# NethermindEth/cairo_zstd

Hardware: NVIDIA B200
Metric: decompressed GB/s (device-timed, whole box) at 1/2/4/8 B200; % of HBM roofline (higher is better)
Workload: dtype u8

## Files before the change

cairo_zstd_b200/csrc/czb_internal.cuh:

```cuda
#pragma once
#include <cuda_runtime.h>
#include <stdint.h>

#include "../../include/cairo_zstd_b200.h"


namespace czb {

constexpr uint32_t NONE32 = 0xFFFFFFFFu;
constexpr uint32_t MAX_BLOCK_SIZE = 128u * 1024u;
constexpr uint64_t MAX_FRAME_OUT = 0x0FFFFFFEull;

enum : uint8_t { BT_RAW = 0, BT_RLE = 1, BT_COMPRESSED = 2, BT_ERROR = 3 };
enum : uint8_t { LT_RAW = 0, LT_RLE = 1, LT_COMPRESSED = 2, LT_TREELESS = 3 };
enum : uint8_t { MODE_PREDEFINED = 0, MODE_RLE = 1, MODE_FSE = 2, MODE_REPEAT = 3 };

struct FrameInfo {
    int32_t status;
    uint32_t hdr_len;
    uint64_t fcs;
    uint64_t window;
    uint8_t descriptor;
    uint8_t has_checksum;
    uint16_t pad0;
    uint32_t checksum;
    uint32_t n_blocks;
    uint32_t n_huf;
    uint32_t n_fse;
    uint32_t size_cls;
    uint64_t lit_bytes;
    uint64_t n_seq;
    uint64_t n_seq_true;
    uint64_t src_end;
    uint32_t block_base;
    uint32_t fse_cls;
};

struct __align__(16) BlockDesc {
    uint32_t frame;
    uint32_t src_off;
    uint32_t size;
    uint8_t type;
    uint8_t last;
    uint8_t lit_type;
    uint8_t n_streams;
    int32_t pre_status;
    int32_t seqhdr_status;
    uint32_t regen;
    uint32_t lit_src_off;
    uint32_t lit_comp;
    uint32_t huf_src_blk;
    uint64_t lit_off;
    uint32_t n_seq;
    uint32_t seq_src_off;
    uint32_t seq_src_len;
    uint8_t modes;
    uint8_t first_in_frame;
    uint16_t pad;
    uint64_t seq_off;
    uint32_t tbl_src_blk[3];
    int32_t huf_status;
    int32_t fse_status;
    uint32_t hist_out[3];
    uint32_t out_bytes;
    uint32_t ml_sum;
};
static_assert(sizeof(BlockDesc) == 112, "BlockDesc layout");
constexpr uint32_t SEQ_ALIGN = 4;
__host__ __device__ inline uint64_t seq_slots(uint64_t n_seq) { return (n_seq + SEQ_ALIGN - 1) & ~(uint64_t)(SEQ_ALIGN - 1); }

typedef unsigned long long Seq;
constexpr uint32_t OFF29_CLAMP = (1u << 28) - 1u;
__host__ __device__ inline uint32_t seq_ll(Seq r) { return (uint32_t)r & 0x1FFFFu; }
__host__ __device__ inline uint32_t seq_ml(Seq r) { return (uint32_t)(r >> 17) & 0x3FFFFu; }
__host__ __device__ inline uint32_t seq_off29(Seq r) { return (uint32_t)(r >> 35); }

constexpr uint32_t SYM_BASE = 0xF0000000u;
constexpr uint32_t SYM_MID = 0x00800000u;
constexpr uint32_t REAL_OFF_CLAMP = 0xEFFFFFFFu;
__host__ __device__ inline uint32_t sym_enc(uint32_t k) { return SYM_BASE + (k << 24) + SYM_MID; }
__host__ __device__ inline bool sym_is(uint32_t v) { return v >= SYM_BASE; }
__host__ __device__ inline uint32_t sym_resolve(uint32_t v, uint32_t h0, uint32_t h1, uint32_t h2) {
    uint32_t t = v - SYM_BASE;
    uint32_t k = t >> 24;
    uint32_t c = SYM_MID - (t & 0x00FFFFFFu);
    uint32_t base = k == 0 ? h0 : (k == 1 ? h1 : h2);
    return base - c;
}
__host__ __device__ inline uint32_t off29_pack(uint32_t v) {
    if (v >= SYM_BASE) { uint32_t t = v - SYM_BASE; return (1u << 28) | ((t >> 24) << 24) | (SYM_MID - (t & 0x00FFFFFFu)); }
    return v < OFF29_CLAMP ? v : OFF29_CLAMP;
}
__host__ __device__ inline uint32_t off29_resolve(uint32_t f, uint32_t h0, uint32_t h1, uint32_t h2) {
    if (f >> 28) { uint32_t k = (f >> 24) & 3u, c = f & 0x00FFFFFFu; return (k == 0 ? h0 : (k == 1 ? h1 : h2)) - c; }
    return f;
}

struct FrameResume {
    uint32_t start_block;
    uint32_t h0, h1, h2;
    uint64_t out0;
    uint64_t bytes_read0;
};

struct WaveCounters {
    unsigned long long n_blocks, lit_bytes, n_seq;
    unsigned int n_huf, n_fse;
    unsigned int n_huf_cls[2];
    unsigned int exec_next;
    unsigned int pad[3];
    unsigned int frame_fill[32];
    unsigned int fse_fill[32];
};

struct HufRec {
    uint8_t weights[256];
    uint16_t nw;
    uint8_t max_bits;
    uint8_t pad;
    uint32_t tree_bytes;
    int32_t status;
    uint32_t blk;
};

struct WaveTotals {
    unsigned long long n_blocks, lit_bytes, n_seq, n_huf, n_fse, src_bytes;
    unsigned int frame_cls[32], fse_cls[32];
};
__host__ __device__ inline uint32_t size_class(uint64_t v) {
    uint32_t c = 0;
    while (v > 1 && c < 31) { v >>= 1; c++; }
    return c;
}

struct RevBits {
    const uint32_t* w0;
    uint32_t lo_mask;
    int wi;
    int avail;
    int rem;
    uint32_t wnext;
    uint64_t buf;

    __device__ __forceinline__ uint32_t load_word(int i) const {
        uint32_t w = 0;
        if (i >= 0) { w = w0[i]; if (i == 0) w &= lo_mask; }
        return w;
    }
    __device__ __forceinline__ void topup() {
        const uint32_t w = wi == -1 ? (wnext & lo_mask) : wnext;
        buf |= (uint64_t)w << (32 - avail);
        avail += 32;
        wnext = 0;
        if (wi >= 0) {
            wnext = w0[wi];
            if (wi >= 32) asm volatile("prefetch.global.L1 [%0];" ::"l"(w0 + wi - 32));
        }
        wi--;
    }
    __device__ __forceinline__ void topup_if_low() { if (avail <= 32) topup(); }
    __device__ __forceinline__ bool init(const uint8_t* p, int n) {
        rem = n * 8; avail = 0; buf = 0; wnext = 0; wi = -3; w0 = nullptr; lo_mask = 0;
        if (n <= 0) return false;
        const uintptr_t a0 = reinterpret_cast<uintptr_t>(p), a_last = a0 + (uintptr_t)n - 1;
        w0 = reinterpret_cast<const uint32_t*>(a0 & ~uintptr_t(3));
        lo_mask = 0xFFFFFFFFu << ((uint32_t)(a0 & 3) * 8);
        const int wl = (int)((a_last - reinterpret_cast<uintptr_t>(w0)) >> 2);
        const uint32_t v = (uint32_t)(a_last & 3) + 1;
        uint32_t w = load_word(wl) << ((4 - v) * 8);
        buf = (uint64_t)w << 32;
        avail = (int)(8 * v);
        wnext = wl - 1 >= 0 ? w0[wl - 1] : 0u;
        wi = wl - 2;
        topup();
        const uint32_t top = (uint32_t)(buf >> 56);
        if (top == 0) return false;
        const int pad = __clz(top) - 24 + 1;
        buf <<= pad; avail -= pad; rem -= pad;
        return true;
    }
    __device__ __forceinline__ uint32_t peek(int n) const {
        return (uint32_t)((buf >> 1) >> (63 - n));
    }
    __device__ __forceinline__ void skip(int n) { buf <<= n; avail -= n; rem -= n; }
    __device__ __forceinline__ uint32_t get(int n) { uint32_t v = peek(n); skip(n); return v; }
    __device__ __forceinline__ uint32_t get_safe(int n) { if (avail < n) topup(); return get(n); }
};

__device__ __forceinline__ void cp_async16(uint32_t smem_addr, const void* g) {
    asm volatile("cp.async.cg.shared.global [%0], [%1], 16;" ::"r"(smem_addr), "l"(g) : "memory");
}
__device__ __forceinline__ void cp_async16_if(bool pred, uint32_t smem_addr, const void* g) {
    asm volatile("{\n\t.reg .pred p;\n\tsetp.ne.u32 p, %2, 0;\n\t@p cp.async.cg.shared.global [%0], [%1], 16;\n\t}" ::"r"(smem_addr), "l"(g), "r"((uint32_t)pred) : "memory");
}
__device__ __forceinline__ void cp_async16_sz(uint32_t smem_addr, const void* g, uint32_t src_bytes) {
    asm volatile("cp.async.cg.shared.global [%0], [%1], 16, %2;" ::"r"(smem_addr), "l"(g), "r"(src_bytes) : "memory");
}
__device__ __forceinline__ void cp_async_commit() { asm volatile("cp.async.commit_group;" ::: "memory"); }
template <int N>
__device__ __forceinline__ void cp_async_wait() { asm volatile("cp.async.wait_group %0;" ::"n"(N) : "memory"); }
__device__ __forceinline__ uint32_t lds32(uint32_t smem_addr) {
    uint32_t v;
    asm volatile("ld.shared.u32 %0, [%1];" : "=r"(v) : "r"(smem_addr) : "memory");
    return v;
}

__device__ __forceinline__ uint32_t shr_clamp(uint32_t x, uint32_t n) {
    uint32_t v;
    asm("shr.b32 %0, %1, %2;" : "=r"(v) : "r"(x), "r"(n));
    return v;
}
template <int RING_BYTES, int WAIT>
struct RevBitsWinT {
    static constexpr int RING = RING_BYTES;
    static constexpr int WAIT_GROUPS = WAIT;
    const uint8_t* c_lo;
    uint32_t ring;
    int P;
    int start;
    int chunk;

    __device__ __forceinline__ int rem() const { return P - start; }
    __device__ __forceinline__ uint32_t window() const {
        const uint32_t wo = ((uint32_t)P >> 5) << 2;
        const uint32_t hi = lds32(ring + (wo & (RING - 1))), lo = lds32(ring + ((wo - 4u) & (RING - 1)));
        return __funnelshift_r(lo, hi, (uint32_t)P & 31u);
    }
    struct Raw { uint32_t lo, hi, sh; };
    __device__ __forceinline__ Raw window_raw() const {
        const uint32_t wo = ((uint32_t)P >> 5) << 2;
        Raw r;
        r.hi = lds32(ring + (wo & (RING - 1))); r.lo = lds32(ring + ((wo - 4u) & (RING - 1))); r.sh = (uint32_t)P & 31u;
        return r;
    }
    static __device__ __forceinline__ uint32_t window_of(const Raw& r) { return __funnelshift_r(r.lo, r.hi, r.sh); }
    struct Raw64 { uint32_t w0, w1, w2, sh; };
    __device__ __forceinline__ Raw64 window64_raw() const {
        const uint32_t wo = ((uint32_t)P >> 5) << 2;
        Raw64 r;
        r.w2 = lds32(ring + (wo & (RING - 1))); r.w1 = lds32(ring + ((wo - 4u) & (RING - 1))); r.w0 = lds32(ring + ((wo - 8u) & (RING - 1)));
        r.sh = (uint32_t)P & 31u;
        return r;
    }
    __device__ __forceinline__ uint32_t window_masked() const {
        uint32_t x = window();
        const int left = P - start;
        if (left < 32) x = left <= 0 ? 0u : (x & ~shr_clamp(0xFFFFFFFFu, (uint32_t)left));
        return x;
    }
    __device__ __forceinline__ void refill() {
        const int cn = (P - 1) >> 7;
        cp_async16_if(cn < chunk && chunk >= RING / 16, ring + (uint32_t)((chunk & (RING / 16 - 1)) << 4), c_lo + ((chunk - RING / 16) << 4));
        chunk = cn;
    }
    __device__ __forceinline__ void refill_nobranch(uint32_t dummy) {
        const int cn = (P - 1) >> 7;
        const bool left = cn < chunk, need = left && chunk >= RING / 16;
        const uint32_t dst = need ? ring + (uint32_t)((chunk & (RING / 16 - 1)) << 4) : dummy;
        cp_async16_sz(dst, c_lo + (need ? ((chunk - RING / 16) << 4) : 0), need ? 16u : 0u);
        chunk -= left ? 1 : 0;
    }
    __device__ __forceinline__ Raw window_raw_at(int Q) const {
        const uint32_t wo = ((uint32_t)Q >> 5) << 2;
        Raw r;
        r.hi = lds32(ring + (wo & (RING - 1))); r.lo = lds32(ring + ((wo - 4u) & (RING - 1))); r.sh = (uint32_t)Q & 31u;
        return r;
    }
    __device__ __forceinline__ void step_sync() { cp_async_commit(); cp_async_wait<WAIT_GROUPS>(); }
    __device__ __forceinline__ uint32_t get(int n) {
        uint32_t x = window();
        const int left = P - start;
        if (left < 32) x = left <= 0 ? 0u : (x & ~shr_clamp(0xFFFFFFFFu, (uint32_t)left));
        const uint32_t v = shr_clamp(x, 32u - (uint32_t)n);
        P -= n;
        refill();
        return v;
    }
    __device__ __forceinline__ bool init(const uint8_t* p, int n, uint32_t ring_smem_addr) {
        c_lo = p; ring = ring_smem_addr; P = 0; start = 0; chunk = 0;
        if (n <= 0) return false;
        const uintptr_t a0 = reinterpret_cast<uintptr_t>(p);
        c_lo = reinterpret_cast<const uint8_t*>(a0 & ~uintptr_t(15));
        start = (int)(a0 & 15) * 8;
        const int last = (int)(a0 & 15) + n - 1;
        chunk = last >> 4;
#pragma unroll
        for (int k = 0; k < RING / 16; k++) {
            const int c = chunk - k;
            if (c >= 0) cp_async16(ring + (uint32_t)((c & (RING / 16 - 1)) << 4), c_lo + (c << 4));
        }
        cp_async_commit();
        cp_async_wait<0>();
        P = 8 * (last + 1);
        const uint32_t x = window();
        if ((x >> 24) == 0) return false;
        P -= __clz(x) + 1;
        refill();
        return true;
    }
};
using RevBitsWin = RevBitsWinT<128, 5>;

struct FwdBits {
    const uint8_t* p;
    int len;
    int idx;
    uint64_t w64 = 0;
    int wbyte = -64;
    __device__ __forceinline__ bool get(int n, uint32_t& v) {
        if (len * 8 - idx < n) return false;
        const int byte = idx >> 3;
        if (byte < wbyte || byte + 4 > wbyte + 8) {
            uint64_t w = 0;
#pragma unroll
            for (int k = 0; k < 8; k++) if (byte + k < len) w |= (uint64_t)p[byte + k] << (8 * k);
            w64 = w; wbyte = byte;
        }
        v = (uint32_t)(w64 >> (idx - 8 * wbyte)) & ((1u << n) - 1u);
        idx += n;
        return true;
    }
};

__device__ __forceinline__ uint32_t highest_bit_set(uint32_t v) { return v ? 32u - (uint32_t)__clz(v) : 0u; }
__device__ __forceinline__ unsigned lane_id() { return threadIdx.x & 31u; }
__device__ __forceinline__ unsigned lanemask_lt() { unsigned m; asm("mov.u32 %0, %%lanemask_lt;" : "=r"(m)); return m; }

struct LaunchCtx { cudaStream_t stream; uint64_t* launches; };

void launch_scan_frames(const LaunchCtx& lc, const czb_frame_desc* descs, FrameInfo* infos, uint64_t n,
                        uint64_t wave_frames, WaveTotals* totals, const FrameResume* resume);
void launch_wave_totals(const LaunchCtx& lc, const FrameInfo* infos, uint64_t n, uint64_t wave_frames, WaveTotals* totals,
                        uint64_t n_waves);
void launch_fill_blocks(const LaunchCtx& lc, const czb_frame_desc* descs, FrameInfo* infos, uint64_t first, uint64_t count,
                        BlockDesc* blocks, uint32_t* huf_items, uint32_t* fse_items, WaveCounters* counters,
                        const WaveTotals* wave_totals, uint32_t* exec_order, int exact_fse_classes, const FrameResume* resume);
void launch_huff(const LaunchCtx& lc, const czb_frame_desc* descs, BlockDesc* blocks, const uint32_t* items,
                 WaveCounters* counters, uint32_t max_items, uint8_t* lit_scratch, HufRec* recs, uint32_t* cls_items0,
                 uint32_t* cls_items1, void* big_weight_scratch);
uint64_t huff_big_scratch_bytes();
void launch_dict_parse(const LaunchCtx& lc, const uint8_t* raw, uint64_t len, czb_dictionary_info* out, void* big_weight_scratch);
void launch_fse(const LaunchCtx& lc, const czb_frame_desc* descs, BlockDesc* blocks, const uint32_t* items,
                const WaveCounters* counters, uint32_t max_items, Seq* seq_scratch);
struct BigRule { uint32_t big_cls, big_seq_bytes, share_cls; uint64_t share_bytes; };
struct ExecSide { cudaStream_t stream; cudaEvent_t fork, join; bool flow, flow_wide; const FrameResume* resume; };
void launch_exec_flow(const LaunchCtx& lc, unsigned n_ctas, const czb_frame_desc* descs, const FrameInfo* infos, BigRule rule, const uint32_t* exec_order,
                      BlockDesc* blocks, const uint8_t* lit_scratch, const Seq* seq_scratch, czb_frame_result* results, const FrameResume* resume,
                      bool wide);
void launch_exec(const LaunchCtx& lc, const ExecSide& side, int sm_count, const czb_frame_desc* descs, const FrameInfo* infos, uint64_t first, uint64_t count, uint32_t n_big_cls,
                 uint32_t n_exec, BigRule rule, WaveCounters* counters,
                 const uint32_t* exec_order, BlockDesc* blocks, const uint8_t* lit_scratch, const Seq* seq_scratch,
                 czb_frame_result* results);
void launch_xxh64(const LaunchCtx& lc, const czb_frame_desc* descs, czb_frame_result* results, uint64_t first, uint64_t count);
void launch_publish_totals(const LaunchCtx& lc, const WaveTotals* totals_d, WaveTotals* totals_host_mapped, uint64_t n_waves);
void launch_header_results(const LaunchCtx& lc, const FrameInfo* infos, czb_frame_result* results, uint64_t n);
void launch_frame_sizes(const LaunchCtx& lc, const FrameInfo* infos, uint64_t first, uint64_t count, const BlockDesc* blocks,
                        czb_frame_result* results);
void launch_split_frames(const LaunchCtx& lc, const uint8_t* buf, uint64_t len, czb_frame_span* spans, uint64_t cap, unsigned long long* counts);
int setup_kernel_attributes();

}
```

cairo_zstd_b200/csrc/k_huff.cu:

```cuda
#include "czb_fse_build.cuh"
#include "czb_internal.cuh"

namespace czb {

constexpr int HUF_WARPS = 2;
constexpr int HUF_SLOTS_PER_WARP = 8;
constexpr int HUF_SLOTS = HUF_WARPS * HUF_SLOTS_PER_WARP;
constexpr int HUF_MAX_LOG = 11;
constexpr int HUF_SMALL_LOG = 9;
constexpr int HUF_PREP_WARPS = 4;
constexpr int HUF_SMALL_SMEM_PERCENT = 100;

struct HufSlot {
    const uint8_t* data;
    uint8_t* dst;
    uint32_t off[4];
    uint32_t len[4];
    uint32_t expect[4];
    uint32_t dst_off[4];
    uint32_t max_bits;
    uint32_t n_streams;
    uint32_t regen;
    uint32_t blk;
    int32_t status;
};

struct HufWarpTmp {
    uint8_t weights[264];
    uint8_t sorted[264];
    uint32_t cnt[16];
    uint32_t cell0[16];
    uint32_t sort0[16];
    uint32_t run[16];
    int16_t probs[FSE_MAX_SYMBOLS];
    uint8_t rank_sym[1 << FSE_MAX_LOG];
};

using HufBits = RevBitsWinT<64, 5>;

template <int LOG>
struct HufSmem {
    uint16_t table[HUF_SLOTS][1 << LOG];
    HufSlot slot[HUF_SLOTS];
    union alignas(16) WarpScratch {
        HufWarpTmp tmp;
        uint8_t ring[32][HufBits::RING];
    } scratch[HUF_WARPS];
};

struct HufPrepSmem {
    uint16_t fse_table[HUF_PREP_WARPS][1 << FSE_MAX_LOG];
    HufWarpTmp tmp[HUF_PREP_WARPS];
};

__device__ __noinline__ int32_t huf_read_weights_big(const uint8_t* fs, uint32_t fslen, uint32_t header, HufWarpTmp& t, FseBigScratch* big,
                                                     uint32_t& n_weights) {
    const unsigned lane = lane_id();
    if (lane == 0) { while (atomicCAS(&big->lock, 0, 1) != 0) __nanosleep(200); }
    __syncwarp();
    __threadfence();
    int n_probs = 0, log = 0, used = 0;
    int32_t st = CZS_OK;
    if (lane == 0) st = fse_read_probabilities(fs, (int)fslen, 100, t.probs, n_probs, log, used, big->probs);
    st = __shfl_sync(0xFFFFFFFFu, st, 0);
    used = __shfl_sync(0xFFFFFFFFu, used, 0);
    n_probs = __shfl_sync(0xFFFFFFFFu, n_probs, 0);
    log = __shfl_sync(0xFFFFFFFFu, log, 0);
    uint32_t nw = 0;
    if (st == CZS_OK) {
        __threadfence();
        __syncwarp();
        fse_build_table_big(big->probs, n_probs, log, big->table, big->rank_sym);
        __threadfence();
        __syncwarp();
        if ((uint32_t)used > header) st = CZS_HUF_FSE_TABLE_USED_TOO_MANY_BYTES;
        else if (lane == 0) {
            const uint32_t clen = header - (uint32_t)used;
            const uint32_t* tab = big->table;
            RevBits br;
            if (!br.init(fs + used, (int)clen)) st = CZS_HUF_EXTRA_PADDING;
            else {
                const uint32_t size = 1u << log;
                auto rd = [&](uint32_t n) -> uint32_t { uint32_t v = 0; while (n) { const uint32_t k = n > 16u ? 16u : n; v = (v << k) | br.get_safe((int)k); n -= k; } return v; };
                uint32_t e1 = tab[rd((uint32_t)log)];
                uint32_t e2 = tab[rd((uint32_t)log)];
                for (;;) {
                    if (nw < 264) t.weights[nw] = (uint8_t)fse_big_sym(e1);
                    nw++;
                    uint32_t nb = fse_big_nbits(e1, log);
                    e1 = tab[(fse_big_base(e1, nb, log) + rd(nb)) & (size - 1)];
                    if (br.rem <= -1) { if (nw < 264) t.weights[nw] = (uint8_t)fse_big_sym(e2); nw++; break; }
                    if (nw < 264) t.weights[nw] = (uint8_t)fse_big_sym(e2);
                    nw++;
                    nb = fse_big_nbits(e2, log);
                    e2 = tab[(fse_big_base(e2, nb, log) + rd(nb)) & (size - 1)];
                    if (br.rem <= -1) { if (nw < 264) t.weights[nw] = (uint8_t)fse_big_sym(e1); nw++; break; }
                    if (nw > 255) { st = CZS_HUF_TOO_MANY_WEIGHTS; break; }
                }
            }
        }
    }
    __syncwarp();
    st = __shfl_sync(0xFFFFFFFFu, st, 0);
    n_weights = __shfl_sync(0xFFFFFFFFu, nw, 0);
    __threadfence();
    if (lane == 0) atomicExch(&big->lock, 0);
    __syncwarp();
    return st;
}

__device__ int32_t huf_read_weights(const uint8_t* p, uint32_t len, HufWarpTmp& t, uint16_t* fse_table, uint32_t& n_weights,
                                    uint32_t& bytes_used, FseBigScratch* big) {
    const unsigned lane = lane_id();
    if (len == 0) return CZS_HUF_SOURCE_IS_EMPTY;
    const uint32_t header = p[0];
    if (header <= 127) {
        const uint8_t* fs = p + 1;
        const uint32_t fslen = len - 1;
        if (header > fslen) return CZS_HUF_NOT_ENOUGH_BYTES_FOR_WEIGHTS;
        if (big && fslen >= 1 && 5u + (fs[0] & 15u) > (uint32_t)FSE_MAX_LOG) {
            const int32_t stb = huf_read_weights_big(fs, fslen, header, t, big, n_weights);
            bytes_used = 1 + header;
            return stb;
        }
        int n_probs = 0, log = 0, used = 0;
        int32_t st = CZS_OK;
        if (lane == 0) st = fse_read_probabilities(fs, (int)fslen, 100, t.probs, n_probs, log, used);
        st = __shfl_sync(0xFFFFFFFFu, st, 0);
        used = __shfl_sync(0xFFFFFFFFu, used, 0);
        if (st == CZS_UNSUPPORTED && (uint32_t)used > header) return CZS_HUF_FSE_TABLE_USED_TOO_MANY_BYTES;
        if (st != CZS_OK) return st;
        n_probs = __shfl_sync(0xFFFFFFFFu, n_probs, 0);
        log = __shfl_sync(0xFFFFFFFFu, log, 0);
        __syncwarp();
        fse_build_table_warp(t.probs, n_probs, log, fse_table, t.rank_sym);
        __syncwarp();
        if ((uint32_t)used > header) return CZS_HUF_FSE_TABLE_USED_TOO_MANY_BYTES;
        const uint32_t clen = header - (uint32_t)used;
        uint32_t nw = 0;
        if (lane == 0) {
            RevBits br;
            if (!br.init(fs + used, (int)clen)) st = CZS_HUF_EXTRA_PADDING;
            else {
                const uint32_t size = 1u << log;
                uint32_t e1 = fse_table[br.get_safe(log)];
                uint32_t e2 = fse_table[br.get_safe(log)];
                for (;;) {
                    br.topup_if_low();
                    if (nw < 264) t.weights[nw] = (uint8_t)fse_entry_sym(e1);
                    nw++;
                    uint32_t nb = fse_entry_nbits(e1, log);
                    e1 = fse_table[(fse_entry_base(e1, nb, log) + br.get(nb)) & (size - 1)];
                    if (br.rem <= -1) { if (nw < 264) t.weights[nw] = (uint8_t)fse_entry_sym(e2); nw++; break; }
                    if (nw < 264) t.weights[nw] = (uint8_t)fse_entry_sym(e2);
                    nw++;
                    nb = fse_entry_nbits(e2, log);
                    e2 = fse_table[(fse_entry_base(e2, nb, log) + br.get(nb)) & (size - 1)];
                    if (br.rem <= -1) { if (nw < 264) t.weights[nw] = (uint8_t)fse_entry_sym(e1); nw++; break; }
                    if (nw > 255) { st = CZS_HUF_TOO_MANY_WEIGHTS; break; }
                }
            }
        }
        st = __shfl_sync(0xFFFFFFFFu, st, 0);
        n_weights = __shfl_sync(0xFFFFFFFFu, nw, 0);
        bytes_used = 1 + header;
        __syncwarp();
        return st;
    }
    const uint32_t nw = header - 127;
    const uint32_t need = (nw + 1) / 2;
    if (len - 1 < need) return CZS_HUF_NOT_ENOUGH_BYTES_IN_SOURCE;
    for (uint32_t i = lane; i < nw; i += 32) {
        const uint8_t b = p[1 + i / 2];
        t.weights[i] = (i & 1) ? (b & 0xF) : (b >> 4);
    }
    n_weights = nw;
    bytes_used = 1 + need;
    __syncwarp();
    return CZS_OK;
}

__device__ int32_t huf_check_weights(HufWarpTmp& t, uint32_t nw, uint32_t& max_bits_out) {
    const unsigned lane = lane_id();
    uint32_t sum = 0;
    bool too_big = false;
    for (uint32_t i = lane; i < nw; i += 32) {
        const uint32_t w = t.weights[i];
        if (w > 11) too_big = true;
        else if (w) sum += 1u << (w - 1);
    }
    if (__any_sync(0xFFFFFFFFu, too_big)) return CZS_HUF_WEIGHT_BIGGER_THAN_MAX_NUM_BITS;
#pragma unroll
    for (int o = 16; o > 0; o >>= 1) sum += __shfl_xor_sync(0xFFFFFFFFu, sum, o);
    if (sum == 0) return CZS_HUF_MISSING_WEIGHTS;
    const uint32_t max_bits = highest_bit_set(sum);
    const uint32_t left_over = (1u << max_bits) - sum;
    if (left_over & (left_over - 1)) return CZS_HUF_LEFTOVER_NOT_POWER_OF_2;
    const uint32_t last_weight = highest_bit_set(left_over);
    max_bits_out = max_bits;
    if (max_bits > 11) return CZS_HUF_MAX_BITS_TOO_HIGH;
    if (nw >= 256) return CZS_PANIC_INTERNAL;
    if (lane == 0) t.weights[nw] = (uint8_t)last_weight;
    __syncwarp();
    return CZS_OK;
}

__device__ void huf_fill_table(HufWarpTmp& t, uint32_t nw, uint32_t max_bits, uint16_t* table) {
    const unsigned lane = lane_id();
    if (lane < 16) { t.cnt[lane] = 0; t.run[lane] = 0; }
    __syncwarp();
    const uint32_t nsym = nw + 1;
    for (uint32_t s0 = 0; s0 < nsym; s0 += 32) {
        const uint32_t s = s0 + lane;
        const uint32_t w = s < nsym ? t.weights[s] : 0;
        const uint32_t b = w ? max_bits + 1 - w : 0;
        const unsigned same = __match_any_sync(0xFFFFFFFFu, b);
        if (b && (same & lanemask_lt()) == 0) t.cnt[b] += __popc(same);
        __syncwarp();
    }
    if (lane == 0) {
        uint32_t cell = 0, srt = 0;
        for (uint32_t b = max_bits; b >= 1; b--) {
            t.cell0[b] = cell; t.sort0[b] = srt;
            cell += t.cnt[b] << (max_bits - b);
            srt += t.cnt[b];
        }
        t.cell0[0] = cell;
    }
    __syncwarp();
    for (uint32_t s0 = 0; s0 < nsym; s0 += 32) {
        const uint32_t s = s0 + lane;
        const uint32_t w = s < nsym ? t.weights[s] : 0;
        const uint32_t b = w ? max_bits + 1 - w : 0;
        const unsigned same = __match_any_sync(0xFFFFFFFFu, b);
        const uint32_t before = __popc(same & lanemask_lt());
        if (b) t.sorted[t.sort0[b] + t.run[b] + before] = (uint8_t)s;
        __syncwarp();
        if (b && before == 0) t.run[b] += __popc(same);
        __syncwarp();
    }
    const uint32_t size = 1u << max_bits;
    for (uint32_t i = lane; i < size; i += 32) {
        uint32_t b = max_bits;
        while (b > 1 && i >= t.cell0[b - 1]) b--;
        const uint32_t k = (i - t.cell0[b]) >> (max_bits - b);
        table[i] = (uint16_t)(((uint32_t)t.sorted[t.sort0[b] + k] << 8) | b);
    }
    __syncwarp();
}

__global__ void __launch_bounds__(HUF_PREP_WARPS * 32) k_huff_prep(const czb_frame_desc* __restrict__ descs, BlockDesc* __restrict__ blocks,
                                                                    const uint32_t* __restrict__ items, WaveCounters* __restrict__ counters,
                                                                    HufRec* __restrict__ recs, uint32_t* __restrict__ cls_items0,
                                                                    uint32_t* __restrict__ cls_items1, FseBigScratch* __restrict__ big) {
    __shared__ HufPrepSmem sm;
    const uint32_t n_items = counters->n_huf;
    const unsigned warp = threadIdx.x >> 5, lane = lane_id();
    const uint32_t item = blockIdx.x * HUF_PREP_WARPS + warp;
    if (item >= n_items) return;
    HufWarpTmp& tmp = sm.tmp[warp];
    const uint32_t bi = items[item];
    const BlockDesc d = blocks[bi];
    const uint8_t* fsrc = descs[d.frame].src;
    int32_t st = CZS_OK;
    uint32_t nw = 0, tree_bytes = 0, max_bits = 0;
    if (d.lit_type == LT_COMPRESSED) {
        st = huf_read_weights(fsrc + d.lit_src_off, d.lit_comp, tmp, sm.fse_table[warp], nw, tree_bytes, big);
    } else if (d.huf_src_blk == NONE32) {
        st = CZS_UNINITIALIZED_HUFFMAN_TABLE;
    } else {
        const BlockDesc sd = blocks[d.huf_src_blk];
        uint32_t ignored = 0;
        st = huf_read_weights(fsrc + sd.lit_src_off, sd.lit_comp, tmp, sm.fse_table[warp], nw, ignored, big);
    }
    if (st == CZS_OK) st = huf_check_weights(tmp, nw, max_bits);
    HufRec& r = recs[item];
    if (st == CZS_OK) for (uint32_t i = lane; i <= nw; i += 32) r.weights[i] = tmp.weights[i];
    if (lane == 0) {
        r.nw = (uint16_t)nw; r.max_bits = (uint8_t)max_bits; r.tree_bytes = tree_bytes; r.status = st; r.blk = bi;
        if (st != CZS_OK) blocks[bi].huf_status = st;
        else if (max_bits <= HUF_SMALL_LOG) cls_items0[atomicAdd(&counters->n_huf_cls[0], 1u)] = item;
        else cls_items1[atomicAdd(&counters->n_huf_cls[1], 1u)] = item;
    }
}

__device__ __noinline__ void huf_decode_concatenated(const HufSlot& sl, const uint16_t* table) {
    uint32_t pos = 0;
    const int mb = (int)sl.max_bits;
    for (uint32_t q = 0; q < sl.n_streams; q++) {
        RevBits br;
        if (!br.init(sl.data + sl.off[q], (int)sl.len[q])) return;
        while (br.rem > 0) {
            br.topup_if_low();
            const uint32_t e = table[br.peek(mb)];
            br.skip((int)(e & 0xFFu));
            if (pos < sl.regen) sl.dst[pos] = (uint8_t)(e >> 8);
            pos++;
        }
    }
}

template <int LOG>
__global__ void __launch_bounds__(HUF_WARPS * 32) k_huff(const czb_frame_desc* __restrict__ descs, BlockDesc* __restrict__ blocks,
                                                       const uint32_t* __restrict__ items, const HufRec* __restrict__ recs,
                                                       const WaveCounters* __restrict__ counters, int cls,
                                                       uint8_t* __restrict__ lit_scratch) {
    extern __shared__ __align__(16) uint8_t smem_raw[];
    HufSmem<LOG>& sm = *reinterpret_cast<HufSmem<LOG>*>(smem_raw);
    const uint32_t n_items = counters->n_huf_cls[cls];
    const unsigned warp = threadIdx.x >> 5, lane = lane_id();
    const uint32_t first = (blockIdx.x * HUF_WARPS + warp) * HUF_SLOTS_PER_WARP;
    if (first >= n_items) return;
    HufWarpTmp& tmp = sm.scratch[warp].tmp;

    for (int s = 0; s < HUF_SLOTS_PER_WARP; s++) {
        const uint32_t item = first + s;
        HufSlot& sl = sm.slot[warp * HUF_SLOTS_PER_WARP + s];
        uint16_t* table = sm.table[warp * HUF_SLOTS_PER_WARP + s];
        if (item >= n_items) { if (lane == 0) { sl.status = CZS_NOT_DECODED; sl.n_streams = 0; sl.blk = NONE32; } continue; }
        const HufRec& rec = recs[items[item]];
        const uint32_t bi = rec.blk;
        const BlockDesc d = blocks[bi];
        const uint8_t* fsrc = descs[d.frame].src;
        const uint8_t* payload = fsrc + d.lit_src_off;
        uint32_t plen = d.lit_comp;
        int32_t st = CZS_OK;
        const uint32_t max_bits = rec.max_bits, nw = rec.nw, tree_bytes = rec.tree_bytes;
        for (uint32_t i = lane; i <= nw; i += 32) tmp.weights[i] = rec.weights[i];
        __syncwarp();
        huf_fill_table(tmp, nw, max_bits, table);
        if (lane == 0) {
            sl.blk = bi; sl.max_bits = max_bits; sl.n_streams = d.n_streams; sl.regen = d.regen;
            sl.dst = lit_scratch + d.lit_off;
            const uint8_t* data = payload + tree_bytes;
            uint32_t dlen = plen - tree_bytes;
            if (st == CZS_OK) {
                if (d.n_streams == 4) {
                    if (dlen < 6) st = CZS_MISSING_BYTES_FOR_JUMP_HEADER;
                    else {
                        const uint32_t j1 = data[0] | ((uint32_t)data[1] << 8);
                        const uint32_t j2 = j1 + (data[2] | ((uint32_t)data[3] << 8));
                        const uint32_t j3 = j2 + (data[4] | ((uint32_t)data[5] << 8));
                        data += 6; dlen -= 6;
                        if (dlen < j3) st = CZS_MISSING_BYTES_FOR_LITERALS;
                        else {
                            sl.off[0] = 0; sl.len[0] = j1; sl.off[1] = j1; sl.len[1] = j2 - j1;
                            sl.off[2] = j2; sl.len[2] = j3 - j2; sl.off[3] = j3; sl.len[3] = dlen - j3;
                            const uint32_t seg = (d.regen + 3) / 4;
                            for (uint32_t k = 0; k < 4; k++) {
                                const uint32_t start = k * seg;
                                sl.dst_off[k] = start;
                                sl.expect[k] = start >= d.regen ? 0u : (d.regen - start < seg ? d.regen - start : seg);
                            }
                        }
                    }
                } else {
                    sl.off[0] = 0; sl.len[0] = dlen; sl.dst_off[0] = 0; sl.expect[0] = d.regen;
                }
            }
            sl.data = data;
            sl.status = st;
        }
        __syncwarp();
    }
    __syncwarp();

    const int sidx = warp * HUF_SLOTS_PER_WARP + (lane >> 2);
    const unsigned k = lane & 3;
    const HufSlot& sl = sm.slot[sidx];
    const uint16_t* table = sm.table[sidx];
    int32_t my_status = CZS_OK;
    uint32_t produced = 0;
    const bool live = sl.status == CZS_OK && k < sl.n_streams;
    if (live) {
        HufBits br;
        if (!br.init(sl.data + sl.off[k], (int)sl.len[k], (uint32_t)__cvta_generic_to_shared(sm.scratch[warp].ring[lane]))) my_status = CZS_LIT_EXTRA_PADDING;
        else {
            const uint32_t mb = sl.max_bits, s = 32u - mb;
            const uint32_t expect = sl.expect[k];
            uint8_t* wp = sl.dst + sl.dst_off[k];
            uint32_t n = 0;
            auto one = [&]() {
                br.step_sync();
                const uint32_t e = table[br.window_masked() >> s];
                br.P -= (int)(e & 0xFFu);
                br.refill();
                if (n < expect) wp[n] = (uint8_t)(e >> 8);
                n++;
            };
            HufBits::Raw64 w = {0u, 0u, 0u, 0u};
            auto four = [&]() -> uint32_t {
                br.step_sync();
                uint32_t xh = __funnelshift_r(w.w1, w.w2, w.sh), xl = __funnelshift_r(w.w0, w.w1, w.sh);
                const uint32_t e0 = table[xh >> s]; xh = __funnelshift_l(xl, xh, e0); xl = __funnelshift_l(0u, xl, e0);
                const uint32_t e1 = table[xh >> s]; xh = __funnelshift_l(xl, xh, e1); xl = __funnelshift_l(0u, xl, e1);
                const uint32_t e2 = table[xh >> s]; xh = __funnelshift_l(xl, xh, e2);
                const uint32_t e3 = table[xh >> s];
                const uint32_t used = (e0 & 0xFFu) + (e1 & 0xFFu) + (e2 & 0xFFu) + (e3 & 0xFFu);
                br.P -= (int)used;
                br.refill();
                w = br.window64_raw();
                return __byte_perm(__byte_perm(e0, e1, 0x0051), __byte_perm(e2, e3, 0x0051), 0x5410);
            };
            const uint32_t head = (16u - (uint32_t)(reinterpret_cast<uintptr_t>(wp) & 15u)) & 15u;
            while (br.rem() > 0 && n < head) one();
            w = br.window64_raw();
            while (br.rem() >= 176 && n + 16 <= expect) {
                uint4 v;
                v.x = four(); v.y = four(); v.z = four(); v.w = four();
                *reinterpret_cast<uint4*>(wp + n) = v;
                n += 16;
            }
            while (br.rem() >= 44 && n + 4 <= expect) {
                *reinterpret_cast<uint32_t*>(wp + n) = four();
                n += 4;
            }
            while (br.rem() > 0) one();
            produced = n;
            if (sl.n_streams == 4 && br.rem() != 0) my_status = CZS_BITSTREAM_READ_MISMATCH;
        }
    }
    const unsigned base = lane & ~3u;
    int32_t st = CZS_OK;
    uint32_t total = 0;
    bool canonical = true;
#pragma unroll
    for (int q = 0; q < 4; q++) {
        const int32_t sq = __shfl_sync(0xFFFFFFFFu, my_status, base + q);
        const uint32_t pq = __shfl_sync(0xFFFFFFFFu, produced, base + q);
        if (st == CZS_OK && sq != CZS_OK) st = sq;
        total += pq;
        if ((uint32_t)q < sl.n_streams && pq != sl.expect[q]) canonical = false;
    }
    if (k == 0 && sl.blk != NONE32) {
        int32_t fin = sl.status;
        if (fin == CZS_OK) fin = st;
        if (fin == CZS_OK && total != sl.regen) fin = CZS_DECODED_LITERAL_COUNT_MISMATCH;
        if (fin == CZS_OK && !canonical) huf_decode_concatenated(sl, table);
        blocks[sl.blk].huf_status = fin;
    }
}

void launch_huff(const LaunchCtx& lc, const czb_frame_desc* descs, BlockDesc* blocks, const uint32_t* items,
                 WaveCounters* counters, uint32_t max_items, uint8_t* lit_scratch, HufRec* recs, uint32_t* cls_items0,
                 uint32_t* cls_items1, void* big_weight_scratch) {
    if (!max_items) return;
    k_huff_prep<<<(max_items + HUF_PREP_WARPS - 1) / HUF_PREP_WARPS, HUF_PREP_WARPS * 32, 0, lc.stream>>>(descs, blocks, items, counters, recs,
                                                                                                         cls_items0, cls_items1,
                                                                                                         static_cast<FseBigScratch*>(big_weight_scratch));
    ++*lc.launches;
    const unsigned grid = (max_items + HUF_SLOTS - 1) / HUF_SLOTS;
    k_huff<HUF_SMALL_LOG><<<grid, HUF_WARPS * 32, sizeof(HufSmem<HUF_SMALL_LOG>), lc.stream>>>(descs, blocks, cls_items0, recs, counters, 0, lit_scratch);
    ++*lc.launches;
    k_huff<HUF_MAX_LOG><<<grid, HUF_WARPS * 32, sizeof(HufSmem<HUF_MAX_LOG>), lc.stream>>>(descs, blocks, cls_items1, recs, counters, 1, lit_scratch);
    ++*lc.launches;
}

struct DictParseSmem {
    uint16_t huf_table[1 << HUF_MAX_LOG];
    uint16_t fse_table[1 << FSE_MAX_LOG];
    HufWarpTmp tmp;
};
__global__ void __launch_bounds__(32) k_dict_parse(const uint8_t* __restrict__ raw, uint64_t len, czb_dictionary_info* __restrict__ out,
                                                   FseBigScratch* __restrict__ big) {
    __shared__ DictParseSmem sm;
    const unsigned lane = lane_id();
    czb_dictionary_info info;
    memset(&info, 0, sizeof info);
    info.offset_hist[0] = 2; info.offset_hist[1] = 4; info.offset_hist[2] = 8;
    int32_t st = CZS_OK;
    uint32_t h = 2166136261u;
    auto rd32 = [&](uint64_t o) { return (uint32_t)raw[o] | ((uint32_t)raw[o + 1] << 8) | ((uint32_t)raw[o + 2] << 16) | ((uint32_t)raw[o + 3] << 24); };
    uint64_t pos = 8;
    if (len < 8) st = CZS_PANIC_TRUNCATED;
    else if (rd32(0) != 0xEC30A437u) st = CZS_DICT_BAD_MAGIC;
    else info.id = rd32(4);
    if (st == CZS_OK) {
        uint32_t nw = 0, tree_bytes = 0, max_bits = 0;
        st = huf_read_weights(raw + pos, (uint32_t)(len - pos < 0xFFFFFFFFull ? len - pos : 0xFFFFFFFFull), sm.tmp, sm.fse_table, nw, tree_bytes, big);
        if (st == CZS_OK) st = huf_check_weights(sm.tmp, nw, max_bits);
        if (st == CZS_OK) {
            huf_fill_table(sm.tmp, nw, max_bits, sm.huf_table);
            __syncwarp();
            if (lane == 0) for (uint32_t i = 0; i < (1u << max_bits); i++) { const uint32_t e = sm.huf_table[i]; h = (h ^ (((e & 0xFFu) << 8) | (e >> 8))) * 16777619u; }
            info.huf_bytes = tree_bytes; info.huf_max_bits = max_bits; info.n_weights = nw;
            pos += tree_bytes;
        }
    }
    uint32_t used3[3] = {0, 0, 0}, log3[3] = {0, 0, 0};
    for (int k = 0; k < 3 && st == CZS_OK; k++) {
        int n_probs = 0, log = 0, used = 0;
        int32_t pst = CZS_OK;
        if (lane == 0) pst = fse_read_probabilities(raw + pos, (int)(len - pos < 0x7FFFFFFFull ? len - pos : 0x7FFFFFFFull), k == 0 ? 8 : 9, sm.tmp.probs, n_probs, log, used);
        pst = __shfl_sync(0xFFFFFFFFu, pst, 0); n_probs = __shfl_sync(0xFFFFFFFFu, n_probs, 0);
        log = __shfl_sync(0xFFFFFFFFu, log, 0); used = __shfl_sync(0xFFFFFFFFu, used, 0);
        __syncwarp();
        if (pst != CZS_OK) { st = pst; break; }
        fse_build_table_warp(sm.tmp.probs, n_probs, log, sm.fse_table, sm.tmp.rank_sym);
        __syncwarp();
        if (lane == 0) {
            for (uint32_t i = 0; i < (1u << log); i++) {
                const uint32_t e = sm.fse_table[i], nb = fse_entry_nbits(e, (uint32_t)log);
                h = (h ^ (fse_entry_sym(e) | (nb << 8) | (fse_entry_base(e, nb, (uint32_t)log) << 12))) * 16777619u;
            }
        }
        __syncwarp();
        used3[k] = (uint32_t)used; log3[k] = (uint32_t)log;
        pos += (uint64_t)used;
    }
    if (st == CZS_OK) {
        info.of_bytes = used3[0]; info.ml_bytes = used3[1]; info.ll_bytes = used3[2];
        info.of_log = log3[0]; info.ml_log = log3[1]; info.ll_log = log3[2];
        if (len - pos < 12) st = CZS_PANIC_TRUNCATED;
        else {
            info.offset_hist[0] = rd32(pos); info.offset_hist[1] = rd32(pos + 4); info.offset_hist[2] = rd32(pos + 8);
            info.content_off = pos + 12; info.content_len = len - pos - 12;
        }
    }
    if (lane == 0) {
        if (st != CZS_OK) {
            const uint32_t id = info.id;
            memset(&info, 0, sizeof info);
            (void)id;
        } else info.table_hash = h;
        info.status = st;
        *out = info;
    }
}
void launch_dict_parse(const LaunchCtx& lc, const uint8_t* raw, uint64_t len, czb_dictionary_info* out, void* big_weight_scratch) {
    k_dict_parse<<<1, 32, 0, lc.stream>>>(raw, len, out, static_cast<FseBigScratch*>(big_weight_scratch));
    ++*lc.launches;
}

uint64_t huff_big_scratch_bytes() { return sizeof(FseBigScratch); }

int setup_huff_attributes() {
    int rc = (int)cudaFuncSetAttribute(k_huff<HUF_SMALL_LOG>, cudaFuncAttributeMaxDynamicSharedMemorySize, (int)sizeof(HufSmem<HUF_SMALL_LOG>));
    if (rc) return rc;
    cudaFuncSetAttribute(k_huff<HUF_SMALL_LOG>, cudaFuncAttributePreferredSharedMemoryCarveout, HUF_SMALL_SMEM_PERCENT);
    return (int)cudaFuncSetAttribute(k_huff<HUF_MAX_LOG>, cudaFuncAttributeMaxDynamicSharedMemorySize, (int)sizeof(HufSmem<HUF_MAX_LOG>));
}

}
```

Measured before the change: 335.5.

## Parse Huffman weights one item per lane with warp fallback; incremental 64-bit window

Huffman prep now gives each lane its own block and parses small FSE-compressed or direct weight headers in per-lane shared tables, so one warp handles 32 items instead of one. Items the lane path cannot handle (larger table logs, more symbols, errors) fall back to the existing warp-cooperative parser, one at a time. The hot decode loop also updates its three-word bit window incrementally, reloading only the words that changed instead of re-reading all three from shared memory each step. The cost is serial per-lane parsing with divergence, and a fallback path that runs serially inside the warp.

```diff
diff --git a/cairo_zstd_b200/csrc/czb_internal.cuh b/cairo_zstd_b200/csrc/czb_internal.cuh
--- a/cairo_zstd_b200/csrc/czb_internal.cuh
+++ b/cairo_zstd_b200/csrc/czb_internal.cuh
@@ -241,6 +241,16 @@
         r.w2 = lds32(ring + (wo & (RING - 1))); r.w1 = lds32(ring + ((wo - 4u) & (RING - 1))); r.w0 = lds32(ring + ((wo - 8u) & (RING - 1)));
         r.sh = (uint32_t)P & 31u;
         return r;
+    }
+    __device__ __forceinline__ void window64_advance(Raw64& r, int P_old) const {
+        const uint32_t knew = (uint32_t)P >> 5, d = ((uint32_t)P_old >> 5) - knew;
+        r.sh = (uint32_t)P & 31u;
+        if (d != 0) {
+            const uint32_t lo = lds32(ring + ((knew * 4u - 8u) & (RING - 1)));
+            if (d == 1) { r.w2 = r.w1; r.w1 = r.w0; }
+            else { r.w2 = r.w0; r.w1 = lds32(ring + ((knew * 4u - 4u) & (RING - 1))); }
+            r.w0 = lo;
+        }
     }
     __device__ __forceinline__ uint32_t window_masked() const {
         uint32_t x = window();
diff --git a/cairo_zstd_b200/csrc/k_huff.cu b/cairo_zstd_b200/csrc/k_huff.cu
--- a/cairo_zstd_b200/csrc/k_huff.cu
+++ b/cairo_zstd_b200/csrc/k_huff.cu
@@ -48,9 +48,14 @@
     } scratch[HUF_WARPS];
 };
 
+constexpr int HUF_LANE_LOG = 6;
+constexpr int HUF_LANE_SYMBOLS = 12;
+
 struct HufPrepSmem {
-    uint16_t fse_table[HUF_PREP_WARPS][1 << FSE_MAX_LOG];
-    HufWarpTmp tmp[HUF_PREP_WARPS];
+    union {
+        struct { uint16_t table[1 << HUF_LANE_LOG][32]; int16_t probs[HUF_LANE_SYMBOLS][32]; } lane;
+        struct { uint16_t fse_table[1 << FSE_MAX_LOG]; HufWarpTmp tmp; } warp;
+    } w[HUF_PREP_WARPS];
 };
 
 __device__ __noinline__ int32_t huf_read_weights_big(const uint8_t* fs, uint32_t fslen, uint32_t header, HufWarpTmp& t, FseBigScratch* big,
@@ -249,6 +254,147 @@
     __syncwarp();
 }
 
+__device__ bool huf_weights_lane(const uint8_t* p, uint32_t len, uint16_t (*table)[32], int16_t (*probs)[32], unsigned lane,
+                                 uint8_t* w_out, uint32_t& nw_out, uint32_t& bytes_used, uint32_t& max_bits_out) {
+    if (len == 0) return false;
+    const uint32_t header = p[0];
+    uint32_t nw = 0, sum = 0;
+    bool too_big = false;
+    auto put = [&](uint32_t w) {
+        if (nw < 256) w_out[nw] = (uint8_t)w;
+        too_big |= w > 11;
+        sum += w ? 1u << ((w - 1) & 15u) : 0u;
+        nw++;
+    };
+    if (header <= 127) {
+        const uint8_t* fs = p + 1;
+        const uint32_t fslen = len - 1;
+        if (fslen == 0 || header > fslen) return false;
+        FwdBits fb{fs, (int)fslen, 0};
+        uint32_t v;
+        if (!fb.get(4, v) || 5 + (int)v > HUF_LANE_LOG) return false;
+        const int log = 5 + (int)v;
+        const uint32_t size = 1u << log;
+        uint32_t counter = 0;
+        int n = 0;
+        while (counter < size) {
+            const uint32_t max_remaining = size - counter + 1;
+            const int bits = (int)highest_bit_set(max_remaining);
+            uint32_t unchecked;
+            if (!fb.get(bits, unchecked)) return false;
+            const uint32_t low_threshold = ((1u << bits) - 1u) - max_remaining;
+            const uint32_t mask = (1u << (bits - 1)) - 1u;
+            const uint32_t small = unchecked & mask;
+            uint32_t value;
+            if (small < low_threshold) { fb.idx -= 1; value = small; }
+            else if (unchecked > mask) value = unchecked - low_threshold;
+            else value = unchecked;
+            const int prob = (int)value - 1;
+            if (n >= HUF_LANE_SYMBOLS) return false;
+            probs[n++][lane] = (int16_t)prob;
+            if (prob != 0) {
+                counter += prob > 0 ? (uint32_t)prob : 1u;
+            } else {
+                for (;;) {
+                    uint32_t skip;
+                    if (!fb.get(2, skip)) return false;
+                    if (n + (int)skip > HUF_LANE_SYMBOLS) return false;
+                    for (uint32_t k = 0; k < skip; k++) probs[n++][lane] = 0;
+                    if (skip != 3) break;
+                }
+            }
+        }
+        if (counter != size) return false;
+        const uint32_t used = (uint32_t)(fb.idx + 7) >> 3;
+        if (used > header) return false;
+        uint32_t neg = size;
+        for (int s = 0; s < n; s++) if (probs[s][lane] == -1) table[--neg][lane] = fse_entry((uint32_t)s, 1u);
+        const uint32_t step = (size >> 1) + (size >> 3) + 3, cmask = size - 1;
+        uint32_t pos = 0;
+        for (int s = 0; s < n; s++) {
+            for (int k = 0, pr = probs[s][lane]; k < pr; k++) {
+                table[pos][lane] = (uint16_t)((uint32_t)s << 10);
+                do pos = (pos + step) & cmask; while (pos >= neg);
+            }
+        }
+        for (uint32_t i = 0; i < neg; i++) {
+            const uint32_t s = (uint32_t)table[i][lane] >> 10;
+            const int ns = probs[s][lane];
+            probs[s][lane] = (int16_t)(ns + 1);
+            table[i][lane] = fse_entry(s, (uint32_t)ns);
+        }
+        RevBits br;
+        if (!br.init(fs + used, (int)(header - used))) return false;
+        uint32_t e1 = table[br.get_safe(log)][lane];
+        uint32_t e2 = table[br.get_safe(log)][lane];
+        for (;;) {
+            br.topup_if_low();
+            put(fse_entry_sym(e1));
+            uint32_t nb = fse_entry_nbits(e1, (uint32_t)log);
+            e1 = table[(fse_entry_base(e1, nb, (uint32_t)log) + br.get((int)nb)) & cmask][lane];
+            if (br.rem <= -1) { put(fse_entry_sym(e2)); break; }
+            put(fse_entry_sym(e2));
+            nb = fse_entry_nbits(e2, (uint32_t)log);
+            e2 = table[(fse_entry_base(e2, nb, (uint32_t)log) + br.get((int)nb)) & cmask][lane];
+            if (br.rem <= -1) { put(fse_entry_sym(e1)); break; }
+            if (nw > 255) return false;
+        }
+        bytes_used = 1 + header;
+    } else {
+        const uint32_t n = header - 127, need = (n + 1) / 2;
+        if (len - 1 < need) return false;
+        for (uint32_t i = 0; i < n; i++) {
+            const uint8_t b = p[1 + i / 2];
+            put((i & 1) ? (b & 0xFu) : (uint32_t)(b >> 4));
+        }
+        bytes_used = 1 + need;
+    }
+    if (too_big || sum == 0 || nw >= 256) return false;
+    const uint32_t max_bits = highest_bit_set(sum);
+    const uint32_t left_over = (1u << max_bits) - sum;
+    if ((left_over & (left_over - 1)) || max_bits > 11) return false;
+    w_out[nw] = (uint8_t)highest_bit_set(left_over);
+    nw_out = nw;
+    max_bits_out = max_bits;
+    return true;
+}
+
+__device__ __forceinline__ void huf_file_section(uint32_t item, uint32_t max_bits, WaveCounters* counters, uint32_t* cls_items0,
+                                                 uint32_t* cls_items1) {
+    if (max_bits <= HUF_SMALL_LOG) cls_items0[atomicAdd(&counters->n_huf_cls[0], 1u)] = item;
+    else cls_items1[atomicAdd(&counters->n_huf_cls[1], 1u)] = item;
+}
+
+__device__ void huf_prep_warp(uint32_t item, const czb_frame_desc* __restrict__ descs, BlockDesc* __restrict__ blocks,
+                              const uint32_t* __restrict__ items, WaveCounters* __restrict__ counters, HufRec* __restrict__ recs,
+                              uint32_t* __restrict__ cls_items0, uint32_t* __restrict__ cls_items1, FseBigScratch* __restrict__ big,
+                              HufWarpTmp& tmp, uint16_t* fse_table) {
+    const unsigned lane = lane_id();
+    const uint32_t bi = items[item];
+    const BlockDesc d = blocks[bi];
+    const uint8_t* fsrc = descs[d.frame].src;
+    int32_t st = CZS_OK;
+    uint32_t nw = 0, tree_bytes = 0, max_bits = 0;
+    if (d.lit_type == LT_COMPRESSED) {
+        st = huf_read_weights(fsrc + d.lit_src_off, d.lit_comp, tmp, fse_table, nw, tree_bytes, big);
+    } else if (d.huf_src_blk == NONE32) {
+        st = CZS_UNINITIALIZED_HUFFMAN_TABLE;
+    } else {
+        const BlockDesc sd = blocks[d.huf_src_blk];
+        uint32_t ignored = 0;
+        st = huf_read_weights(fsrc + sd.lit_src_off, sd.lit_comp, tmp, fse_table, nw, ignored, big);
+    }
+    if (st == CZS_OK) st = huf_check_weights(tmp, nw, max_bits);
+    HufRec& r = recs[item];
+    if (st == CZS_OK) for (uint32_t i = lane; i <= nw; i += 32) r.weights[i] = tmp.weights[i];
+    if (lane == 0) {
+        r.nw = (uint16_t)nw; r.max_bits = (uint8_t)max_bits; r.tree_bytes = tree_bytes; r.status = st; r.blk = bi;
+        if (st != CZS_OK) blocks[bi].huf_status = st;
+        else huf_file_section(item, max_bits, counters, cls_items0, cls_items1);
+    }
+    __syncwarp();
+}
+
 __global__ void __launch_bounds__(HUF_PREP_WARPS * 32) k_huff_prep(const czb_frame_desc* __restrict__ descs, BlockDesc* __restrict__ blocks,
                                                                     const uint32_t* __restrict__ items, WaveCounters* __restrict__ counters,
                                                                     HufRec* __restrict__ recs, uint32_t* __restrict__ cls_items0,
@@ -256,32 +402,29 @@
     __shared__ HufPrepSmem sm;
     const uint32_t n_items = counters->n_huf;
     const unsigned warp = threadIdx.x >> 5, lane = lane_id();
-    const uint32_t item = blockIdx.x * HUF_PREP_WARPS + warp;
-    if (item >= n_items) return;
-    HufWarpTmp& tmp = sm.tmp[warp];
-    const uint32_t bi = items[item];
-    const BlockDesc d = blocks[bi];
-    const uint8_t* fsrc = descs[d.frame].src;
-    int32_t st = CZS_OK;
-    uint32_t nw = 0, tree_bytes = 0, max_bits = 0;
-    if (d.lit_type == LT_COMPRESSED) {
-        st = huf_read_weights(fsrc + d.lit_src_off, d.lit_comp, tmp, sm.fse_table[warp], nw, tree_bytes, big);
-    } else if (d.huf_src_blk == NONE32) {
-        st = CZS_UNINITIALIZED_HUFFMAN_TABLE;
-    } else {
-        const BlockDesc sd = blocks[d.huf_src_blk];
-        uint32_t ignored = 0;
-        st = huf_read_weights(fsrc + sd.lit_src_off, sd.lit_comp, tmp, sm.fse_table[warp], nw, ignored, big);
-    }
-    if (st == CZS_OK) st = huf_check_weights(tmp, nw, max_bits);
-    HufRec& r = recs[item];
-    if (st == CZS_OK) for (uint32_t i = lane; i <= nw; i += 32) r.weights[i] = tmp.weights[i];
-    if (lane == 0) {
-        r.nw = (uint16_t)nw; r.max_bits = (uint8_t)max_bits; r.tree_bytes = tree_bytes; r.status = st; r.blk = bi;
-        if (st != CZS_OK) blocks[bi].huf_status = st;
-        else if (max_bits <= HUF_SMALL_LOG) cls_items0[atomicAdd(&counters->n_huf_cls[0], 1u)] = item;
-        else cls_items1[atomicAdd(&counters->n_huf_cls[1], 1u)] = item;
-    }
+    const uint32_t first = (blockIdx.x * HUF_PREP_WARPS + warp) * 32;
+    if (first >= n_items) return;
+    const uint32_t item = first + lane;
+    bool done = false;
+    if (item < n_items) {
+        const uint32_t bi = items[item];
+        const BlockDesc& d = blocks[bi];
+        const uint32_t src_blk = d.lit_type == LT_COMPRESSED ? bi : d.huf_src_blk;
+        if (src_blk != NONE32) {
+            const BlockDesc& sd = blocks[src_blk];
+            HufRec& r = recs[item];
+            uint32_t nw = 0, tree_bytes = 0, max_bits = 0;
+            done = huf_weights_lane(descs[d.frame].src + sd.lit_src_off, sd.lit_comp, sm.w[warp].lane.table, sm.w[warp].lane.probs, lane,
+                                    r.weights, nw, tree_bytes, max_bits);
+            if (done) {
+                r.nw = (uint16_t)nw; r.max_bits = (uint8_t)max_bits; r.tree_bytes = src_blk == bi ? tree_bytes : 0u; r.status = CZS_OK; r.blk = bi;
+                huf_file_section(item, max_bits, counters, cls_items0, cls_items1);
+            }
+        }
+    }
+    for (unsigned rest = __ballot_sync(0xFFFFFFFFu, item < n_items && !done); rest; rest &= rest - 1)
+        huf_prep_warp(first + (__ffs(rest) - 1), descs, blocks, items, counters, recs, cls_items0, cls_items1, big, sm.w[warp].warp.tmp,
+                      sm.w[warp].warp.fse_table);
 }
 
 __device__ __noinline__ void huf_decode_concatenated(const HufSlot& sl, const uint16_t* table) {
@@ -397,9 +540,10 @@
                 const uint32_t e2 = table[xh >> s]; xh = __funnelshift_l(xl, xh, e2);
                 const uint32_t e3 = table[xh >> s];
                 const uint32_t used = (e0 & 0xFFu) + (e1 & 0xFFu) + (e2 & 0xFFu) + (e3 & 0xFFu);
+                const int P_old = br.P;
                 br.P -= (int)used;
                 br.refill();
-                w = br.window64_raw();
+                br.window64_advance(w, P_old);
                 return __byte_perm(__byte_perm(e0, e1, 0x0051), __byte_perm(e2, e3, 0x0051), 0x5410);
             };
             const uint32_t head = (16u - (uint32_t)(reinterpret_cast<uintptr_t>(wp) & 15u)) & 15u;
@@ -445,7 +589,7 @@
                  WaveCounters* counters, uint32_t max_items, uint8_t* lit_scratch, HufRec* recs, uint32_t* cls_items0,
                  uint32_t* cls_items1, void* big_weight_scratch) {
     if (!max_items) return;
-    k_huff_prep<<<(max_items + HUF_PREP_WARPS - 1) / HUF_PREP_WARPS, HUF_PREP_WARPS * 32, 0, lc.stream>>>(descs, blocks, items, counters, recs,
+    k_huff_prep<<<(max_items + HUF_PREP_WARPS * 32 - 1) / (HUF_PREP_WARPS * 32), HUF_PREP_WARPS * 32, 0, lc.stream>>>(descs, blocks, items, counters, recs,
                                                                                                          cls_items0, cls_items1,
                                                                                                          static_cast<FseBigScratch*>(big_weight_scratch));
     ++*lc.launches;
```

Result: faster. 344.1, median of 6 (+2.6%).
